# XuanchenLi/Topo4D

Measured on AMD Instinct MI355X. Metric: rasterizer fwd+bwd views/sec, higher is better.
Workload: dtype f32

## Files before the change

topo4d_amd/csrc/t4d_raster_render_bwd.h:

```cpp
template <bool NINE>
__device__ __forceinline__ float reduce10_row(float (&r)[10])
{
    float o2, o5, ta, tb;
#define T4D_RED_HEAD                                                                                  \
        "s_nop 1\n\t"                                                                                 \
        "v_add_f32_dpp %[r0], %[r0], %[r0] row_ror:8 row_mask:0xf bank_mask:0xf\n\t"                  \
        "v_add_f32_dpp %[o2], %[r2], %[r2] row_ror:8 row_mask:0xf bank_mask:0xf\n\t"                  \
        "v_add_f32_dpp %[r4], %[r4], %[r4] row_ror:8 row_mask:0xf bank_mask:0xf\n\t"                  \
        "v_add_f32_dpp %[r6], %[r6], %[r6] row_ror:8 row_mask:0xf bank_mask:0xf\n\t"                  \
        "v_add_f32_dpp %[r8], %[r8], %[r8] row_ror:8 row_mask:0xf bank_mask:0xf\n\t"                  \
        "v_add_f32_dpp %[r0], %[r1], %[r1] row_ror:8 row_mask:0xf bank_mask:0xc\n\t"                  \
        "v_add_f32_dpp %[o2], %[r3], %[r3] row_ror:8 row_mask:0xf bank_mask:0xc\n\t"                  \
        "v_add_f32_dpp %[r4], %[r5], %[r5] row_ror:8 row_mask:0xf bank_mask:0xc\n\t"                  \
        "v_add_f32_dpp %[r6], %[r7], %[r7] row_ror:8 row_mask:0xf bank_mask:0xc\n\t"
#define T4D_RED_TAIL                                                                                  \
        "v_add_f32_dpp %[r1], %[r0], %[r0] row_shl:4 row_mask:0xf bank_mask:0x5\n\t"                  \
        "v_add_f32_dpp %[r3], %[r4], %[r4] row_shl:4 row_mask:0xf bank_mask:0x5\n\t"                  \
        "v_add_f32_dpp %[o5], %[r8], %[r8] row_shl:4 row_mask:0xf bank_mask:0x5\n\t"                  \
        "v_add_f32_dpp %[r1], %[o2], %[o2] row_shr:4 row_mask:0xf bank_mask:0xa\n\t"                  \
        "v_add_f32_dpp %[r3], %[r6], %[r6] row_shr:4 row_mask:0xf bank_mask:0xa\n\t"                  \
        "v_add_f32_dpp %[o5], %[r8], %[r8] row_shr:4 row_mask:0xf bank_mask:0xa\n\t"                  \
        "v_cndmask_b32_e64 %[tb], %[r3], %[r1], %[m1]\n\t"               \
        "v_cndmask_b32_e64 %[ta], %[r1], %[r3], %[m1]\n\t"               \
        "v_add_f32_dpp %[o5], %[o5], %[o5] quad_perm:[2,3,0,1] row_mask:0xf bank_mask:0xf\n\t"        \
        "v_add_f32_dpp %[ta], %[tb], %[ta] quad_perm:[2,3,0,1] row_mask:0xf bank_mask:0xf\n\t"        \
        "v_cndmask_b32_e64 %[tb], %[o5], %[ta], %[m0]\n\t"               \
        "v_cndmask_b32_e64 %[ta], %[ta], %[o5], %[m0]\n\t"               \
        "s_nop 0\n\t"                                                                                 \
        "v_add_f32_dpp %[ta], %[tb], %[ta] quad_perm:[1,0,3,2] row_mask:0xf bank_mask:0xf"
#define T4D_RED_OUT [r0] "+v"(r[0]), [r1] "+v"(r[1]), [o2] "=&v"(o2), [r3] "+v"(r[3]), [r4] "+v"(r[4]), [o5] "=&v"(o5), \
                    [r6] "+v"(r[6]), [r8] "+v"(r[8]), [ta] "=&v"(ta), [tb] "=&v"(tb)
#define T4D_RED_MASKS [m1] "s"(0xccccccccccccccccull), [m0] "s"(0xaaaaaaaaaaaaaaaaull)
    if (NINE) {
        asm(T4D_RED_HEAD T4D_RED_TAIL : T4D_RED_OUT : [r2] "v"(r[2]), [r5] "v"(r[5]), [r7] "v"(r[7]), T4D_RED_MASKS);
    } else {
        asm(T4D_RED_HEAD
            "v_add_f32_dpp %[r8], %[r9], %[r9] row_ror:8 row_mask:0xf bank_mask:0xc\n\t"
            T4D_RED_TAIL
            : T4D_RED_OUT : [r2] "v"(r[2]), [r5] "v"(r[5]), [r7] "v"(r[7]), [r9] "v"(r[9]), T4D_RED_MASKS);
    }
    return ta;
#undef T4D_RED_HEAD
#undef T4D_RED_TAIL
#undef T4D_RED_OUT
#undef T4D_RED_MASKS
}

__device__ __forceinline__ int row10_index(const int lane)
{
    const int b0 = lane & 1, b1 = (lane >> 1) & 1, b2 = (lane >> 2) & 1, b3 = (lane >> 3) & 1;
    if (!b0 && !b1) return 2 * b2 + b3;
    if (!b0 && b1) return 4 + 2 * b2 + b3;
    if (b0 && !b1 && !b2) return 8 + b3;
    return -1;
}

__device__ __forceinline__ uint32_t row_max_u32(uint32_t v)
{
    v = max(v, (uint32_t)__builtin_amdgcn_update_dpp(0, (int)v, 0xB1, 0xf, 0xf, true));
    v = max(v, (uint32_t)__builtin_amdgcn_update_dpp(0, (int)v, 0x4E, 0xf, 0xf, true));
    v = max(v, (uint32_t)__builtin_amdgcn_update_dpp(0, (int)v, 0x141, 0xf, 0xf, true));
    v = max(v, (uint32_t)__builtin_amdgcn_update_dpp(0, (int)v, 0x140, 0xf, 0xf, true));
    return v;
}

#ifndef T4D_BWD_WAVES
#define T4D_BWD_WAVES 5
#endif
#ifndef T4D_SEG_WAVES
#define T4D_SEG_WAVES 5
#endif
#ifndef T4D_BWD_DA_WAVES
#define T4D_BWD_DA_WAVES T4D_BWD_WAVES
#endif
#define T4D_BWD_NW (LAT ? 2 : (SEGN != 0 ? T4D_SEG_WAVES : (DA ? T4D_BWD_DA_WAVES : T4D_BWD_WAVES)))
#define T4D_BWD_ATTR __attribute__((amdgpu_waves_per_eu(LAT ? 1 : T4D_BWD_NW, T4D_BWD_NW)))
constexpr int kAcc = 10;
constexpr int kEmptySpan = 64;
template <bool DA, bool LAT, int SEGN, bool LONG = false>
__global__ __launch_bounds__(kBlock) T4D_BWD_ATTR void k_render_bwd(const KP kp)
{
    constexpr bool SEG = SEGN != 0;
    constexpr int kSeg = SEG ? SEGN : ::kSeg;
    constexpr int kBwdBatch = SEG ? SEGN : ::kBwdBatch;
    constexpr int kSlabs = LAT ? 16 : 4;
    constexpr int kChunks = (kBwdBatch + 63) / 64;
    constexpr int kListStride = kBwdBatch + 4;
    constexpr int kEnt = 40;
    static_assert(kBwdBatch % 64 == 0, "staged slots come in chunks of one per lane");
    static_assert(kGP == kAcc, "the slab entry and the scratch record hold the same ten sums");
    static_assert(kAcc * 4 == kEnt, "a slab entry and a staged record must have the same stride");
    struct __attribute__((aligned(16))) Shared {
        unsigned char rec[(kBwdBatch + 1) * kEnt];
        float acc[kSlabs][kBwdBatch + 1][kAcc];
        unsigned short list[4][4][kListStride];
        float cut_r2[kChunks * 64];
        uint32_t pair[kBwdBatch];
        uint32_t wmax[4];
    };
    static_assert(((kBwdBatch + 1) * kEnt) % 8 == 0 && (sizeof(float) * kSlabs * (kBwdBatch + 1) * kAcc) % 8 == 0 &&
                  (sizeof(unsigned short) * 16 * kListStride) % 8 == 0, "8-byte members must stay 8-byte aligned");
    __shared__ Shared sh;
    auto &s_rec = sh.rec;
    auto &s_pair = sh.pair;
    auto &s_acc = sh.acc;
    auto &s_r2 = sh.cut_r2;
    auto &s_wmax = sh.wmax;
    auto &s_list = sh.list;
    constexpr int kNull = kBwdBatch;

    const int tid = threadIdx.x;
    const int wave = tid >> 6, lane = tid & 63, row = lane >> 4;
    const int my_slot = (!DA && row10_index(lane & 15) == 9) ? -1 : row10_index(lane & 15);
    if (tid == 0) {
#pragma unroll
        for (int k = 0; k < kEnt / 8; k++) reinterpret_cast<float2 *>(s_rec + kNull * kEnt)[k] = make_float2(0.f, 0.f);
    }
    if (blockIdx.x >= kp.tile_blocks) {
        const uint32_t spans = (uint32_t)(kp.T + kEmptySpan - 1) / kEmptySpan;
        const uint32_t j = blockIdx.x - kp.tile_blocks;
        const int v = (int)(j / spans), t0 = (int)(j % spans) * kEmptySpan;
        const float *vb = kp.views + (size_t)v * T4D_VIEW_FLOATS + 35;
        const float b0 = vb[0], b1 = vb[1], b2 = vb[2];
        if (b0 == 0.f && b1 == 0.f && b2 == 0.f) return;
        const size_t HWe = (size_t)kp.H * kp.W;
        const float *dc = kp.dL_dcolor + (size_t)v * 3 * HWe;
        for (int t = t0; t < min(t0 + kEmptySpan, kp.T); t++) {
            if (kp.tile_count[(size_t)v * kp.T + t] != 0u) continue;
            const int ty = t / kp.gx, tx = t - ty * kp.gx;
            int ex, ey;
            tile_pixel(tid, tx, ty, ex, ey);
            float d = 0.f;
            if (ex < kp.W && ey < kp.H) {
                const size_t pe = (size_t)ey * kp.W + ex;
                d = fmaf(b0, dc[pe], fmaf(b1, dc[HWe + pe], b2 * dc[2 * HWe + pe]));
            }
            d = wave_sum_to_lane63(d);
            if (lane == 63) kp.tile_dot[((size_t)v * kp.T + t) * 4 + wave] = d;
        }
        return;
    }
    uint4 it;
    if (SEG && !LONG) {
        it = kp.slot_tab[blockIdx.x];
        if (it.w == 0u) return;
    }
    for (int i = tid; i < kSlabs * (kBwdBatch + 1) * kAcc; i += kBlock) (&s_acc[0][0][0])[i] = 0.f;
    for (uint32_t item = blockIdx.x; item < (SEG ? (LONG ? kp.status->live_segments : blockIdx.x + 1u) : (uint32_t)(kp.V * kp.T)); item += kp.tile_blocks) {
    if (SEG && LONG) it = kp.slot_tab[kp.live[item]];
    if (!SEG) it = kp.items[item];
    const int seg_j = SEG ? (int)(it.w & 0x7fffffffu) : 0;
    const int v = (int)(it.x >> 20), t_ = (int)(it.x & 0xfffffu);
    const int ty = t_ / kp.gx, tx = t_ - ty * kp.gx;
    const uint32_t off = it.y, n = it.z;
    if (n == 0) break;
    if (!SEG && LONG && n >= kp.seg_min_pairs &&
        kp.slot_tab[(size_t)v * kp.slots_per_view + seg_slot0(kp, off, (uint32_t)t_)].w != 0u) continue;
    const unsigned long long *keys = kp.keys + (size_t)v * kp.cap + off;
    const float *r2_in = kp.cut_r2 + (size_t)v * kp.cap + off;
    const float2 *xy = kp.xy + (size_t)v * kp.P;
    const float4 *co = kp.conic_opacity + (size_t)v * kp.P;
    const float *rgb = kp.shs ? kp.rgb + (size_t)v * kp.P * 3 : kp.colors_precomp + 3 * param_row0(kp, v);
    const int32_t *radii = kp.radii + (size_t)v * kp.P;
    const uint32_t *pair_off = kp.pair_off + (size_t)v * kp.P;
    float2 *grad_pair = reinterpret_cast<float2 *>(kp.grad_pair) + (size_t)v * kp.cap * (kGP / 2);
    const float *vr = kp.views + (size_t)v * T4D_VIEW_FLOATS;

    int px, py;
    tile_pixel(tid, tx, ty, px, py);
    const bool inside = px < kp.W && py < kp.H;
    const v2f pix_f = { (float)px, (float)py };
    const size_t HW = (size_t)kp.H * kp.W, pix = (size_t)py * kp.W + px;

    float T_final = 0.f, dp0 = 0.f, dp1 = 0.f, dp2 = 0.f, ddep = 0.f, dalp = 0.f;
    uint32_t last_contributor = 0;
    if (inside) {
        T_final = kp.final_T[(size_t)v * HW + pix];
        last_contributor = kp.n_contrib[(size_t)v * HW + pix];
        const float *dc = kp.dL_dcolor + (size_t)v * 3 * HW;
        dp0 = dc[pix]; dp1 = dc[HW + pix]; dp2 = dc[2 * HW + pix];
        if (DA && kp.dL_ddepth) ddep = kp.dL_ddepth[(size_t)v * HW + pix];
        if (DA && kp.dL_dalpha) dalp = kp.dL_dalpha[(size_t)v * HW + pix];
    }
    const v2f dp01 = { dp0, dp1 };
    float T = T_final;
    float acc = vr[35] * dp0 + vr[36] * dp1 + vr[37] * dp2;
    const int nb = (int)((n + kBwdBatch - 1) / kBwdBatch);
    if (SEG && seg_j + 1 < nb) {
        const uint32_t p = (uint32_t)(seg_j + 1) * kSeg;
        if (last_contributor > p) {
            const float *sb = kp.snap + ((size_t)v * kp.slots_per_view + seg_slot0(kp, off, (uint32_t)t_)) * (kSnapFloats * kBlock) + tid;
            const float *sp = sb + (size_t)seg_j * (kSnapFloats * kBlock), *sf = sb + (size_t)(nb - 1) * (kSnapFloats * kBlock);
            const float Tp = sp[0];
            float suf = fmaf(sf[kBlock] - sp[kBlock], dp0, fmaf(sf[2 * kBlock] - sp[2 * kBlock], dp1, (sf[3 * kBlock] - sp[3 * kBlock]) * dp2));
            if (DA) suf = fmaf(sf[4 * kBlock] - sp[4 * kBlock], ddep, suf) + (Tp - T_final) * dalp;
            acc = fmaf(T_final, acc, suf) / Tp;
            T = Tp;
        }
    }

    const uint32_t rmax_v = row_max_u32(last_contributor);
    uint32_t row_max[4];
#pragma unroll
    for (int r = 0; r < 4; r++) row_max[r] = lane_value(rmax_v, 16 * r);
    const uint32_t wave_max = max(max(row_max[0], row_max[1]), max(row_max[2], row_max[3]));
    if (lane == 0) s_wmax[wave] = wave_max;
    __syncthreads();
    const uint32_t tile_max = max(max(s_wmax[0], s_wmax[1]), max(s_wmax[2], s_wmax[3]));

    for (int bi = SEG ? seg_j : nb - 1; bi >= (SEG ? seg_j : 0); bi--) {
        const uint32_t lo = (uint32_t)bi * kBwdBatch;
        const int cnt = (int)min((uint32_t)kBwdBatch, n - lo);
        const bool live = lo < tile_max;
        if (tid < cnt) s_pair[tid] = 0xffffffffu;
        if (tid < kChunks * 64) {
            float r2 = -1.f;
            float2 p = make_float2(0.f, 0.f);
            if (tid < cnt) {
                const unsigned long long key = keys[lo + tid];
                const float r2_kept = live ? r2_in[lo + tid] : -1.f;
                const uint32_t g = (uint32_t)key;
                if (g < (uint32_t)kp.P) {
                    const float2 pg = xy[g];
                    const int rad = radii[g];
                    const uint32_t po = pair_off[g];
                    float4 c = make_float4(0.f, 0.f, 0.f, 0.f);
                    float c0 = 0.f, c1 = 0.f, c2 = 0.f;
                    if (live) { c = co[g]; c0 = rgb[3 * (size_t)g]; c1 = rgb[3 * (size_t)g + 1]; c2 = rgb[3 * (size_t)g + 2]; }
                    p = pg;
                    int x0, y0, x1, y1;
                    tile_rect(pg.x, pg.y, rad, kp.gx, kp.gy, x0, y0, x1, y1);
                    const int local = (ty - y0) * (x1 - x0) + (tx - x0);
                    s_pair[tid] = (tx >= x0 && tx < x1 && ty >= y0 && ty < y1) ? po + (uint32_t)local : 0xffffffffu;
                    if (live) {
                        const float4 q4 = scale_conic(c);
                        float2 *rec = reinterpret_cast<float2 *>(s_rec + tid * kEnt);
                        rec[0] = make_float2(q4.x, q4.y); rec[1] = make_float2(q4.z, q4.w);
                        rec[2] = make_float2(c0, c1);
                        rec[3] = make_float2(c2, __uint_as_float((uint32_t)(key >> 32)));
                        r2 = r2_kept;
                    }
                }
            }
            if (live) {
                reinterpret_cast<float2 *>(s_rec + tid * kEnt)[4] = p;
                s_r2[tid] = r2;
            }
        }
        __syncthreads();
        if (live) {
            unsigned long long mt[4][kChunks];
#pragma unroll
            for (int c2 = 0; c2 < kChunks; c2++) {
                const int slot = (c2 << 6) + lane;
                unsigned long long mc[4] = { 0ull, 0ull, 0ull, 0ull };
                if ((c2 << 6) < cnt)
                    wave_touch_masks(reinterpret_cast<const float2 *>(s_rec + slot * kEnt)[4], s_r2[slot], tx, ty, wave, mc);
#pragma unroll
                for (int r = 0; r < 4; r++) mt[r][c2] = mc[r];
            }
            int nsteps = 0, cnts[4];
#pragma unroll
            for (int r = 0; r < 4; r++) {
                unsigned long long m[kChunks];
#pragma unroll
                for (int c2 = 0; c2 < kChunks; c2++) {
                    m[c2] = mt[r][c2];
                    const uint32_t base = lo + ((uint32_t)c2 << 6);
                    if (row_max[r] <= base) m[c2] = 0;
                    else if (row_max[r] - base < 64u) m[c2] &= (1ull << (row_max[r] - base)) - 1ull;
                }
                cnts[r] = build_visit_list<kChunks, true, kEnt>(m, s_list[wave][r], lane);
                nsteps = max(nsteps, cnts[r]);
            }
#pragma unroll
            for (int r = 0; r < 4; r++) pad_visit_list(s_list[wave][r], cnts[r], nsteps, lane, (unsigned short)(kNull * kEnt));
            __builtin_amdgcn_wave_barrier();
            unsigned long long conflict[kChunks];
#pragma unroll
            for (int c2 = 0; c2 < kChunks; c2++) {
                conflict[c2] = 0ull;
                if (!LAT && (c2 << 6) < nsteps) {
                    const int st = (c2 << 6) + lane;
                    const unsigned short *l0 = s_list[wave][0];
                    const uint32_t e0 = l0[st], e1 = l0[kListStride + st], e2 = l0[2 * kListStride + st], e3 = l0[3 * kListStride + st];
                    const uint32_t nul = (uint32_t)(kNull * kEnt);
                    const bool same = st < nsteps && ((e0 == e1 && e0 != nul) || (e0 == e2 && e0 != nul) || (e0 == e3 && e0 != nul) ||
                                                      (e1 == e2 && e1 != nul) || (e1 == e3 && e1 != nul) || (e2 == e3 && e2 != nul));
                    conflict[c2] = __ballot(same);
                }
            }
            unsigned long long conflict_s[kChunks];
#pragma unroll
            for (int c2 = 0; c2 < kChunks; c2++) conflict_s[c2] = uniform_u64(conflict[c2]);
            const unsigned short *list = s_list[wave][row];
            const unsigned char *rec_b = s_rec;
            unsigned char *slab = LAT ? reinterpret_cast<unsigned char *>(my_slot >= 0 ? &s_acc[wave * 4 + row][0][my_slot]
                                                                                      : &s_acc[wave * 4 + row][kNull][(lane & 15) % kAcc])
                                      : reinterpret_cast<unsigned char *>(&s_acc[wave][0][0] + (my_slot >= 0 ? my_slot : 0));
            const uint32_t slab_and = (!LAT || my_slot >= 0) ? 0xffffffffu : 0u;
            const int lc_rel = (int)min(last_contributor - min(last_contributor, lo), (uint32_t)kBwdBatch) * kEnt;
            uint2 pk = *reinterpret_cast<const uint2 *>(list);
            for (int k = 0; k < nsteps; k += 4) {
                const uint32_t ee[4] = { pk.x & 0xffffu, pk.x >> 16, pk.y & 0xffffu, pk.y >> 16 };
                pk = *reinterpret_cast<const uint2 *>(list + k + 4);
                v2f ds[4];
                float Gs[4], alphas[4];
                float4 cds[4];
                bool contribs[4];
#pragma unroll
                for (int u = 0; u < 4; u++) {
                    const float2 *rec = reinterpret_cast<const float2 *>(rec_b + ee[u]);
                    const float2 q01 = rec[0], q23 = rec[1], c01 = rec[2], c23 = rec[3];
                    ds[u] = *reinterpret_cast<const v2f *>(rec + 4) - pix_f;
                    cds[u] = make_float4(c01.x, c01.y, c23.x, c23.y);
                    float p2;
                    eval_splat(make_float4(q01.x, q01.y, q23.x, q23.y), ds[u], p2, Gs[u], alphas[u]);
                    contribs[u] = (int)ee[u] < lc_rel && !(p2 > 0.0f) && !(alphas[u] < T4D_ALPHA_MIN);
                }
                const uint32_t cbits = (uint32_t)(conflict_s[kChunks == 1 ? 0 : (k >> 6)] >> (k & 63));
#pragma unroll
                for (int u = 0; u < 4; u++) {
                    const bool contrib = contribs[u];
                    const v2f d = ds[u];
                    const float G = Gs[u], alpha = alphas[u];
                    float *dst = reinterpret_cast<float *>(slab + (LAT ? (ee[u] & slab_and) : ee[u]));
                    const float old = *dst;
                    float e = 0.f, w = 0.f;
                    if (LAT) {
                        const float4 cd = cds[u];
                        const float om = 1.f - alpha;
                        const float inv = __builtin_amdgcn_rcpf(om);
                        const float Tn = T * inv;
                        float q = fmaf(cd.x, dp01.x, fmaf(cd.y, dp01.y, cd.z * dp2));
                        if (DA) q = fmaf(cd.w, ddep, q) + dalp;
                        const float qma = q - acc;
                        const float dL_dalpha = qma * Tn;
                        T = contrib ? Tn : T;
                        w = contrib ? alpha * Tn : 0.f;
                        e = contrib ? G * dL_dalpha : 0.f;
                        acc = contrib ? fmaf(alpha, qma, acc) : acc;
                    } else if (contrib) {
                        const float4 cd = cds[u];
                        const float om = 1.f - alpha;
                        const float inv = __builtin_amdgcn_rcpf(om);
                        T = T * inv;
                        w = alpha * T;
                        float q = fmaf(cd.x, dp01.x, fmaf(cd.y, dp01.y, cd.z * dp2));
                        if (DA) q = fmaf(cd.w, ddep, q) + dalp;
                        const float qma = q - acc;
                        const float dL_dalpha = qma * T;
                        e = G * dL_dalpha;
                        acc = fmaf(alpha, qma, acc);
                    }
                    const v2f ed = e * d, edd = ed * d, wdp = w * dp01;
                    float r[10] = { e, ed.x, ed.y, edd.x, ed.x * d.y, edd.y, wdp.x, wdp.y, w * dp2, DA ? w * ddep : 0.f };
                    const float tot = reduce10_row<!DA>(r);
                    const bool add = my_slot >= 0;
                    if (LAT) {
                        *dst = old + tot;
                    } else if (!((cbits >> u) & 1u)) {
                        if (add) *dst = old + tot;
                    } else {
#pragma unroll
                        for (int rr = 0; rr < 4; rr++) {
                            if (add && row == rr) *dst += tot;
                            __builtin_amdgcn_fence(__ATOMIC_RELEASE, "wavefront");
                            __builtin_amdgcn_wave_barrier();
                        }
                    }
                }
            }
        }
        __syncthreads();
        if (tid < cnt) {
            float a[10];
#pragma unroll
            for (int k = 0; k < 10; k++) a[k] = 0.f;
#pragma unroll
            for (int w = 0; w < kSlabs; w++) {
                float2 *src = reinterpret_cast<float2 *>(&s_acc[w][tid][0]);
#pragma unroll
                for (int k = 0; k < 5; k++) {
                    const float2 b2 = src[k];
                    a[2 * k] += b2.x; a[2 * k + 1] += b2.y;
                    src[k] = make_float2(0.f, 0.f);
                }
            }
            const uint32_t pr = s_pair[tid];
            if (pr < kp.cap) {
#pragma unroll
                for (int k = 0; k < kGP / 2; k++) grad_pair[(size_t)pr * (kGP / 2) + k] = make_float2(a[2 * k], a[2 * k + 1]);
            }
        }
        __syncthreads();
    }
    if (kp.tile_dot && seg_j == 0) {
        const float d = wave_sum_to_lane63(acc);
        if (lane == 63) kp.tile_dot[((size_t)v * kp.T + t_) * 4 + wave] = d;
    }
    }
}
```

Baseline: 56230.

## Reduce per-splat gradients as pixel-offset moments and shift about splat centre later

Instead of reducing ten products per splat (e, e*dx, e*dy, e*dx^2, ...) that depend on the splat-to-pixel offset, each row now reduces raw moments of e over fixed pixel coordinates relative to the wave's 8x8 sub-tile centre. The fixed per-lane weights are folded into the DPP reduction, and the moments are converted to offset form once per splat in the flush step, using double-precision shifts with the splat centre. This removes per-contribution multiplies and reduction work from the hot loop. To make it work, the backward pixel mapping is changed, snapshot reads are remapped to forward thread order, and e is truncated (low mantissa bits masked), which adds some precision risk and a more expensive flush.

```diff
diff --git a/topo4d_amd/csrc/t4d_raster_render_bwd.h b/topo4d_amd/csrc/t4d_raster_render_bwd.h
--- a/topo4d_amd/csrc/t4d_raster_render_bwd.h
+++ b/topo4d_amd/csrc/t4d_raster_render_bwd.h
@@ -1,59 +1,108 @@
+__device__ __forceinline__ void tile_pixel_bwd(int tid, int tx, int ty, int &px, int &py)
+{
+    const int w = tid >> 6, r = (tid >> 4) & 3, i = tid & 15;
+    px = tx * T4D_TILE_X + ((w & 1) << 3) + ((r & 1) << 2) + (i >> 2);
+    py = ty * T4D_TILE_Y + ((w >> 1) << 3) + ((r >> 1) << 2) + (i & 3);
+}
+
+__device__ __forceinline__ int fwd_thread_of(int tid) { return (tid & ~15) | ((tid & 3) << 2) | ((tid >> 2) & 3); }
+
+struct RowWeights { float X, ks, kg; };
+
+__device__ __forceinline__ RowWeights row_weights(const int lane)
+{
+    const int r = lane >> 4, i = lane & 15, bank = i >> 2, b1 = (i >> 1) & 1;
+    RowWeights k;
+    k.X = (float)(((r & 1) << 2) + (i >> 2)) - 3.5f;
+    const float y0 = (float)((r >> 1) << 2) - 3.5f;
+    const float Y = y0 + (float)(i & 3), Yp = y0 + (float)((i & 3) ^ 2);
+    auto Ka = [&](float y) { return bank == 1 ? y * y : (bank == 3 ? 0.f : 1.f); };
+    auto Kb = [&](float y) { return (bank & 1) ? 0.f : y; };
+    k.ks = b1 ? Kb(Y) : Ka(Y);
+    k.kg = b1 ? Kb(Yp) : Ka(Yp);
+    return k;
+}
+
 template <bool NINE>
-__device__ __forceinline__ float reduce10_row(float (&r)[10])
-{
-    float o2, o5, ta, tb;
-#define T4D_RED_HEAD                                                                                  \
+__device__ __forceinline__ float reduce_moments_row(const float e, const float ex, const float exx, const float c0, const float c1,
+                                                    const float c2, const float cd, const RowWeights &k)
+{
+    float a, b, c;
+#define T4D_RED_X                                                                                     \
         "s_nop 1\n\t"                                                                                 \
-        "v_add_f32_dpp %[r0], %[r0], %[r0] row_ror:8 row_mask:0xf bank_mask:0xf\n\t"                  \
-        "v_add_f32_dpp %[o2], %[r2], %[r2] row_ror:8 row_mask:0xf bank_mask:0xf\n\t"                  \
-        "v_add_f32_dpp %[r4], %[r4], %[r4] row_ror:8 row_mask:0xf bank_mask:0xf\n\t"                  \
-        "v_add_f32_dpp %[r6], %[r6], %[r6] row_ror:8 row_mask:0xf bank_mask:0xf\n\t"                  \
-        "v_add_f32_dpp %[r8], %[r8], %[r8] row_ror:8 row_mask:0xf bank_mask:0xf\n\t"                  \
-        "v_add_f32_dpp %[r0], %[r1], %[r1] row_ror:8 row_mask:0xf bank_mask:0xc\n\t"                  \
-        "v_add_f32_dpp %[o2], %[r3], %[r3] row_ror:8 row_mask:0xf bank_mask:0xc\n\t"                  \
-        "v_add_f32_dpp %[r4], %[r5], %[r5] row_ror:8 row_mask:0xf bank_mask:0xc\n\t"                  \
-        "v_add_f32_dpp %[r6], %[r7], %[r7] row_ror:8 row_mask:0xf bank_mask:0xc\n\t"
-#define T4D_RED_TAIL                                                                                  \
-        "v_add_f32_dpp %[r1], %[r0], %[r0] row_shl:4 row_mask:0xf bank_mask:0x5\n\t"                  \
-        "v_add_f32_dpp %[r3], %[r4], %[r4] row_shl:4 row_mask:0xf bank_mask:0x5\n\t"                  \
-        "v_add_f32_dpp %[o5], %[r8], %[r8] row_shl:4 row_mask:0xf bank_mask:0x5\n\t"                  \
-        "v_add_f32_dpp %[r1], %[o2], %[o2] row_shr:4 row_mask:0xf bank_mask:0xa\n\t"                  \
-        "v_add_f32_dpp %[r3], %[r6], %[r6] row_shr:4 row_mask:0xf bank_mask:0xa\n\t"                  \
-        "v_add_f32_dpp %[o5], %[r8], %[r8] row_shr:4 row_mask:0xf bank_mask:0xa\n\t"                  \
-        "v_cndmask_b32_e64 %[tb], %[r3], %[r1], %[m1]\n\t"               \
-        "v_cndmask_b32_e64 %[ta], %[r1], %[r3], %[m1]\n\t"               \
-        "v_add_f32_dpp %[o5], %[o5], %[o5] quad_perm:[2,3,0,1] row_mask:0xf bank_mask:0xf\n\t"        \
-        "v_add_f32_dpp %[ta], %[tb], %[ta] quad_perm:[2,3,0,1] row_mask:0xf bank_mask:0xf\n\t"        \
-        "v_cndmask_b32_e64 %[tb], %[o5], %[ta], %[m0]\n\t"               \
-        "v_cndmask_b32_e64 %[ta], %[ta], %[o5], %[m0]\n\t"               \
-        "s_nop 0\n\t"                                                                                 \
-        "v_add_f32_dpp %[ta], %[tb], %[ta] quad_perm:[1,0,3,2] row_mask:0xf bank_mask:0xf"
-#define T4D_RED_OUT [r0] "+v"(r[0]), [r1] "+v"(r[1]), [o2] "=&v"(o2), [r3] "+v"(r[3]), [r4] "+v"(r[4]), [o5] "=&v"(o5), \
-                    [r6] "+v"(r[6]), [r8] "+v"(r[8]), [ta] "=&v"(ta), [tb] "=&v"(tb)
-#define T4D_RED_MASKS [m1] "s"(0xccccccccccccccccull), [m0] "s"(0xaaaaaaaaaaaaaaaaull)
+        "v_add_f32_dpp %[a], %[v0], %[v0] row_ror:8 row_mask:0xf bank_mask:0xf\n\t"                   \
+        "v_add_f32_dpp %[b], %[v2], %[v2] row_ror:8 row_mask:0xf bank_mask:0xf\n\t"                   \
+        "v_add_f32_dpp %[c], %[v4], %[v4] row_ror:8 row_mask:0xf bank_mask:0xf\n\t"                   \
+        "v_add_f32_dpp %[a], %[v1], %[v1] row_ror:8 row_mask:0xf bank_mask:0xc\n\t"                   \
+        "v_add_f32_dpp %[b], %[v3], %[v3] row_ror:8 row_mask:0xf bank_mask:0xc\n\t"                   \
+        "v_add_f32_dpp %[c], %[v5], %[v5] row_ror:8 row_mask:0xf bank_mask:0xc\n\t"
+#define T4D_RED_X4                                                                                    \
+        "v_add_f32_dpp %[a], %[a], %[a] row_shl:4 row_mask:0xf bank_mask:0x5\n\t"                     \
+        "v_add_f32_dpp %[a], %[b], %[b] row_shr:4 row_mask:0xf bank_mask:0xa\n\t"                     \
+        "v_add_f32_dpp %[b], %[c], %[c] row_shl:4 row_mask:0xf bank_mask:0x5\n\t"                     \
+        "v_add_f32_dpp %[b], %[c], %[c] row_shr:4 row_mask:0xf bank_mask:0xa\n\t"
+#define T4D_RED_OUT [a] "=&v"(a), [b] "=&v"(b), [c] "=&v"(c)
+#define T4D_RED_IN [v0] "v"(exx), [v1] "v"(c0), [v2] "v"(c1), [v3] "v"(c2), [v4] "v"(e), [v5] "v"(ex), [ks] "v"(k.ks), [kg] "v"(k.kg), \
+                   [m0] "s"(0xaaaaaaaaaaaaaaaaull)
     if (NINE) {
-        asm(T4D_RED_HEAD T4D_RED_TAIL : T4D_RED_OUT : [r2] "v"(r[2]), [r5] "v"(r[5]), [r7] "v"(r[7]), T4D_RED_MASKS);
+        asm(T4D_RED_X T4D_RED_X4
+            "v_add_f32_dpp %[a], %[a], %[a] quad_perm:[2,3,0,1] row_mask:0xf bank_mask:0xf\n\t"
+            "v_mul_f32_e32 %[c], %[b], %[ks]\n\t"
+            "v_fmac_f32_dpp %[c], %[b], %[kg] quad_perm:[2,3,0,1] row_mask:0xf bank_mask:0xf\n\t"
+            "v_cndmask_b32_e64 %[b], %[a], %[c], %[m0]\n\t"
+            "v_cndmask_b32_e64 %[c], %[c], %[a], %[m0]\n\t"
+            "s_nop 0\n\t"
+            "v_add_f32_dpp %[c], %[b], %[c] quad_perm:[1,0,3,2] row_mask:0xf bank_mask:0xf"
+            : T4D_RED_OUT : T4D_RED_IN);
+        return c;
     } else {
-        asm(T4D_RED_HEAD
-            "v_add_f32_dpp %[r8], %[r9], %[r9] row_ror:8 row_mask:0xf bank_mask:0xc\n\t"
-            T4D_RED_TAIL
-            : T4D_RED_OUT : [r2] "v"(r[2]), [r5] "v"(r[5]), [r7] "v"(r[7]), [r9] "v"(r[9]), T4D_RED_MASKS);
-    }
-    return ta;
-#undef T4D_RED_HEAD
-#undef T4D_RED_TAIL
+        float d;
+        asm(T4D_RED_X
+            "v_add_f32_dpp %[d], %[v6], %[v6] row_ror:8 row_mask:0xf bank_mask:0xf\n\t"
+            T4D_RED_X4
+            "v_add_f32_dpp %[d], %[d], %[d] row_ror:4 row_mask:0xf bank_mask:0xf\n\t"
+            "v_cndmask_b32_e64 %[c], %[d], %[a], %[m1]\n\t"
+            "v_cndmask_b32_e64 %[d], %[a], %[d], %[m1]\n\t"
+            "v_mul_f32_e32 %[a], %[b], %[ks]\n\t"
+            "v_fmac_f32_dpp %[a], %[b], %[kg] quad_perm:[2,3,0,1] row_mask:0xf bank_mask:0xf\n\t"
+            "v_add_f32_dpp %[d], %[c], %[d] quad_perm:[2,3,0,1] row_mask:0xf bank_mask:0xf\n\t"
+            "v_cndmask_b32_e64 %[b], %[d], %[a], %[m0]\n\t"
+            "v_cndmask_b32_e64 %[a], %[a], %[d], %[m0]\n\t"
+            "s_nop 0\n\t"
+            "v_add_f32_dpp %[a], %[b], %[a] quad_perm:[1,0,3,2] row_mask:0xf bank_mask:0xf"
+            : T4D_RED_OUT, [d] "=&v"(d) : T4D_RED_IN, [v6] "v"(cd), [m1] "s"(0xccccccccccccccccull));
+        return a;
+    }
+#undef T4D_RED_X
+#undef T4D_RED_X4
 #undef T4D_RED_OUT
-#undef T4D_RED_MASKS
+#undef T4D_RED_IN
 }
 
 __device__ __forceinline__ int row10_index(const int lane)
 {
-    const int b0 = lane & 1, b1 = (lane >> 1) & 1, b2 = (lane >> 2) & 1, b3 = (lane >> 3) & 1;
-    if (!b0 && !b1) return 2 * b2 + b3;
-    if (!b0 && b1) return 4 + 2 * b2 + b3;
-    if (b0 && !b1 && !b2) return 8 + b3;
-    return -1;
-}
+    const int b0 = lane & 1, b1 = (lane >> 1) & 1, bank = (lane >> 2) & 3;
+    if (!b0) {
+        if (bank == 0) return b1 ? 2 : 0;
+        if (bank == 1) return b1 ? -1 : 5;
+        if (bank == 2) return b1 ? 4 : 1;
+        return -1;
+    }
+    if (!b1) return bank == 0 ? 3 : (bank == 1 ? 7 : (bank == 2 ? 6 : 8));
+    return bank == 0 ? 9 : -1;
+}
+
+__device__ __forceinline__ void moments_about_centre(float (&m)[10], const float pxf, const float pyf)
+{
+    const double px = pxf, py = pyf, M00 = m[0], M10 = m[1], M01 = m[2], M20 = m[3], M11 = m[4], M02 = m[5];
+    const double sx = fma(px, M00, -M10), sy = fma(py, M00, -M01);
+    m[1] = (float)sx; m[2] = (float)sy;
+    m[3] = (float)fma(px, sx, -fma(px, M10, -M20));
+    m[4] = (float)fma(px, sy, -fma(py, M10, -M11));
+    m[5] = (float)fma(py, sy, -fma(py, M01, -M02));
+}
+
+__device__ __forceinline__ float moment_e(const float e) { return __uint_as_float(__float_as_uint(e) & 0xffffffc0u); }
 
 __device__ __forceinline__ uint32_t row_max_u32(uint32_t v)
 {
@@ -110,8 +159,9 @@
     constexpr int kNull = kBwdBatch;
 
     const int tid = threadIdx.x;
-    const int wave = tid >> 6, lane = tid & 63, row = lane >> 4;
+    const int wave = __builtin_amdgcn_readfirstlane(tid >> 6), lane = tid & 63, row = lane >> 4;
     const int my_slot = (!DA && row10_index(lane & 15) == 9) ? -1 : row10_index(lane & 15);
+    const RowWeights rw = row_weights(lane);
     if (tid == 0) {
 #pragma unroll
         for (int k = 0; k < kEnt / 8; k++) reinterpret_cast<float2 *>(s_rec + kNull * kEnt)[k] = make_float2(0.f, 0.f);
@@ -167,7 +217,7 @@
     const float *vr = kp.views + (size_t)v * T4D_VIEW_FLOATS;
 
     int px, py;
-    tile_pixel(tid, tx, ty, px, py);
+    tile_pixel_bwd(tid, tx, ty, px, py);
     const bool inside = px < kp.W && py < kp.H;
     const v2f pix_f = { (float)px, (float)py };
     const size_t HW = (size_t)kp.H * kp.W, pix = (size_t)py * kp.W + px;
@@ -189,7 +239,7 @@
     if (SEG && seg_j + 1 < nb) {
         const uint32_t p = (uint32_t)(seg_j + 1) * kSeg;
         if (last_contributor > p) {
-            const float *sb = kp.snap + ((size_t)v * kp.slots_per_view + seg_slot0(kp, off, (uint32_t)t_)) * (kSnapFloats * kBlock) + tid;
+            const float *sb = kp.snap + ((size_t)v * kp.slots_per_view + seg_slot0(kp, off, (uint32_t)t_)) * (kSnapFloats * kBlock) + fwd_thread_of(tid);
             const float *sp = sb + (size_t)seg_j * (kSnapFloats * kBlock), *sf = sb + (size_t)(nb - 1) * (kSnapFloats * kBlock);
             const float Tp = sp[0];
             float suf = fmaf(sf[kBlock] - sp[kBlock], dp0, fmaf(sf[2 * kBlock] - sp[2 * kBlock], dp1, (sf[3 * kBlock] - sp[3 * kBlock]) * dp2));
@@ -304,7 +354,6 @@
             for (int k = 0; k < nsteps; k += 4) {
                 const uint32_t ee[4] = { pk.x & 0xffffu, pk.x >> 16, pk.y & 0xffffu, pk.y >> 16 };
                 pk = *reinterpret_cast<const uint2 *>(list + k + 4);
-                v2f ds[4];
                 float Gs[4], alphas[4];
                 float4 cds[4];
                 bool contribs[4];
@@ -312,17 +361,16 @@
                 for (int u = 0; u < 4; u++) {
                     const float2 *rec = reinterpret_cast<const float2 *>(rec_b + ee[u]);
                     const float2 q01 = rec[0], q23 = rec[1], c01 = rec[2], c23 = rec[3];
-                    ds[u] = *reinterpret_cast<const v2f *>(rec + 4) - pix_f;
+                    const v2f d = *reinterpret_cast<const v2f *>(rec + 4) - pix_f;
                     cds[u] = make_float4(c01.x, c01.y, c23.x, c23.y);
                     float p2;
-                    eval_splat(make_float4(q01.x, q01.y, q23.x, q23.y), ds[u], p2, Gs[u], alphas[u]);
+                    eval_splat(make_float4(q01.x, q01.y, q23.x, q23.y), d, p2, Gs[u], alphas[u]);
                     contribs[u] = (int)ee[u] < lc_rel && !(p2 > 0.0f) && !(alphas[u] < T4D_ALPHA_MIN);
                 }
                 const uint32_t cbits = (uint32_t)(conflict_s[kChunks == 1 ? 0 : (k >> 6)] >> (k & 63));
 #pragma unroll
                 for (int u = 0; u < 4; u++) {
                     const bool contrib = contribs[u];
-                    const v2f d = ds[u];
                     const float G = Gs[u], alpha = alphas[u];
                     float *dst = reinterpret_cast<float *>(slab + (LAT ? (ee[u] & slab_and) : ee[u]));
                     const float old = *dst;
@@ -353,9 +401,10 @@
                         e = G * dL_dalpha;
                         acc = fmaf(alpha, qma, acc);
                     }
-                    const v2f ed = e * d, edd = ed * d, wdp = w * dp01;
-                    float r[10] = { e, ed.x, ed.y, edd.x, ed.x * d.y, edd.y, wdp.x, wdp.y, w * dp2, DA ? w * ddep : 0.f };
-                    const float tot = reduce10_row<!DA>(r);
+                    e = moment_e(e);
+                    const float ex = e * rw.X;
+                    const v2f wdp = w * dp01;
+                    const float tot = reduce_moments_row<!DA>(e, ex, ex * rw.X, wdp.x, wdp.y, w * dp2, DA ? w * ddep : 0.f, rw);
                     const bool add = my_slot >= 0;
                     if (LAT) {
                         *dst = old + tot;
@@ -377,15 +426,26 @@
             float a[10];
 #pragma unroll
             for (int k = 0; k < 10; k++) a[k] = 0.f;
-#pragma unroll
-            for (int w = 0; w < kSlabs; w++) {
-                float2 *src = reinterpret_cast<float2 *>(&s_acc[w][tid][0]);
-#pragma unroll
-                for (int k = 0; k < 5; k++) {
-                    const float2 b2 = src[k];
-                    a[2 * k] += b2.x; a[2 * k + 1] += b2.y;
-                    src[k] = make_float2(0.f, 0.f);
-                }
+            const float2 pc = live ? reinterpret_cast<const float2 *>(s_rec + tid * kEnt)[4] : make_float2(0.f, 0.f);
+#pragma unroll 1
+            for (int w = 0; w < 4; w++) {
+                float m[10];
+#pragma unroll
+                for (int k = 0; k < 10; k++) m[k] = 0.f;
+#pragma unroll
+                for (int s = 0; s < kSlabs / 4; s++) {
+                    float2 *src = reinterpret_cast<float2 *>(&s_acc[w * (kSlabs / 4) + s][tid][0]);
+#pragma unroll
+                    for (int k = 0; k < 5; k++) {
+                        const float2 b2 = src[k];
+                        m[2 * k] += b2.x; m[2 * k + 1] += b2.y;
+                        src[k] = make_float2(0.f, 0.f);
+                    }
+                }
+                moments_about_centre(m, pc.x - ((float)(tx * T4D_TILE_X + ((w & 1) << 3)) + 3.5f),
+                                        pc.y - ((float)(ty * T4D_TILE_Y + ((w >> 1) << 3)) + 3.5f));
+#pragma unroll
+                for (int k = 0; k < 10; k++) a[k] += m[k];
             }
             const uint32_t pr = s_pair[tid];
             if (pr < kp.cap) {
```

Result: faster. 57450, median of 6 (+2.2%).
